# triq-org/spectroplot-js

Hardware: NVIDIA B200
Metric: Msamples/s rendered to RGBA spectrogram (N=4096) and % of B200 HBM roofline (higher is better)
Workload: dtype f32

## Files before the change

### spectroplot-js_b200/csrc/sp_kernel_r64.cuh

```cuda
#pragma once
#include "sp_prims.cuh"

#ifndef SP_XP
#define SP_XP 0
#endif
#ifndef SP_R64_TMA
#define SP_R64_TMA 1
#endif

namespace sp {

template <int FMT, bool SUB> struct R64Cfg {
    static constexpr int N = 4096, T = 64, STREAMS = 4, FFT_THREADS = T * STREAMS, STORE_THREADS = 128, THREADS = FFT_THREADS + STORE_THREADS;
    static constexpr int STEPS = 4, F = STREAMS * STEPS;
    static constexpr int FFT_REGS = 232, STORE_REGS = 40;
    static constexpr int SWB = SUB ? 8 : sample_width(FMT == FMT_RUNTIME ? CF64 : FMT);
    static constexpr bool OK = SUB || ((FMT != FMT_RUNTIME) && SWB <= 8);
    static constexpr int XP = 66;
    static constexpr int X_BYTES = 64 * XP * 8;
    static constexpr int WIN_PITCH = 64;
    static constexpr int TW_PITCH = 14;
    static constexpr int ST_PITCH = 1026;
    static constexpr int RING = 4;
    static constexpr bool TMA = SP_R64_TMA != 0;
    static constexpr int TILE_BYTES = TMA ? (STORE_THREADS / 32) * 4096 : 0;
    static constexpr size_t SMEM_BYTES = (size_t)STREAMS * X_BYTES + (size_t)F * ST_PITCH * 4 + (size_t)JH_SIZE * 4
                                       + ((SUB || TMA) ? 0 : (size_t)T * WIN_PITCH * 4) + TILE_BYTES + (size_t)T * TW_PITCH * 8 + 1024
                                       + (size_t)F * 2 * 8  + (size_t)2 * F * 8  + 192 + 1024 ;
    static_assert(SMEM_BYTES <= 232448, "render_r64_kernel: dynamic shared memory above the 227 KB an sm_100 CTA may have");
};

__device__ __forceinline__ unsigned lut_at(unsigned lut_base, unsigned word, int j)
{
    const unsigned a = ((j == 0 ? word << 2 : word >> (8 * j - 2)) & 0x3fcu) | lut_base;
    unsigned v;
    asm volatile("ld.shared.u32 %0, [%1];" : "=r"(v) : "r"(a));
    return v;
}

__device__ __forceinline__ void store_row8(uint32_t *rowp, uint4 a, uint4 b, bool aligned)
{
    if (aligned) st_global_256(rowp, a, b);
    else {
        rowp[0] = a.x; rowp[1] = a.y; rowp[2] = a.z; rowp[3] = a.w;
        rowp[4] = b.x; rowp[5] = b.y; rowp[6] = b.z; rowp[7] = b.w;
    }
}

__device__ __forceinline__ void stream_barrier(int stream)
{
    asm volatile("bar.sync %0, 64;" ::"r"(stream + 1) : "memory");
}

template <int FMT, bool SUB, bool OPT = false>
__global__ void __launch_bounds__(384, 1) render_r64_kernel(const Params p, const float2 *__restrict__ tw14, const __grid_constant__ CUtensorMap tmap)
{
    using B = R64Cfg<FMT, SUB>;
    constexpr int N = B::N, T = B::T, F = B::F;
    constexpr bool FLOAT_IN = SUB || FMT == CF32 || FMT == CF64 || FMT == FMT_RUNTIME;
    extern __shared__ __align__(128) unsigned char smem_r64[];
    const unsigned lut_base = (smem_u32(smem_r64) + 1023u) & ~1023u;
    unsigned char *s_x = smem_r64 + (lut_base - smem_u32(smem_r64)) + 1024;
    unsigned *s_lut = reinterpret_cast<unsigned *>(s_x - 1024);
    unsigned char *s_tiles = s_x + B::STREAMS * B::X_BYTES;
    unsigned *s_stage = reinterpret_cast<unsigned *>(s_tiles + B::TILE_BYTES);
    unsigned *s_jh = s_stage + F * B::ST_PITCH;
    float *s_win = reinterpret_cast<float *>(s_jh + JH_SIZE);
    float2 *s_tw = reinterpret_cast<float2 *>(s_win + ((SUB || B::TMA) ? 0 : T * B::WIN_PITCH));
    uint2 *s_mm = reinterpret_cast<uint2 *>(s_tw + T * B::TW_PITCH);
    float2 *s_fmid = reinterpret_cast<float2 *>(s_mm + F * 2);
    uint64_t *s_mbar = reinterpret_cast<uint64_t *>(s_fmid + 2 * F);
    int *s_off = reinterpret_cast<int *>(s_mbar + B::STREAMS);
    uint64_t *s_full = reinterpret_cast<uint64_t *>(s_off + B::STREAMS * 2);
    uint64_t *s_empty = s_full + 2;
    uint64_t *s_tready = s_empty + 2;
    long long *s_ring = reinterpret_cast<long long *>(s_tready + B::RING);
    long long *s_tile0 = s_ring + B::RING;

    const int tid = threadIdx.x;
    const int s = tid >> 6;
    const int t = tid & 63;
    float2 *X = reinterpret_cast<float2 *>(s_x + (size_t)s * B::X_BYTES);
    unsigned char *raw = reinterpret_cast<unsigned char *>(X);
    uint64_t *mbar = s_mbar + s;

    for (int i = tid; i < JH_SIZE; i += B::THREADS) s_jh[i] = 0;
    const int cmax = p.cmap_len - 1;
    const JhConst jc = jh_const(p);
    for (int i = tid; i < 256; i += B::THREADS) s_lut[i] = i <= cmax ? p.lut[jc.rev ? cmax - i : i] : 0u;
    for (int i = tid; i < T * B::TW_PITCH; i += B::THREADS) s_tw[i] = tw14[i];
    if constexpr (!SUB && !B::TMA)
        for (int i = tid; i < N; i += B::THREADS) s_win[(i & 63) * B::WIN_PITCH + (((i >> 6) + 4 * (i & 63)) & 63)] = p.window[i];
    const unsigned jh_base = smem_u32(s_jh) - (JH_MAGIC_BITS << 2);
    const int nfull = p.n_full, sub_r = p.sub_r;

    auto stage = [&](long long xr, int k0sub, unsigned par) {
        if (xr >= p.chunk_frames) xr = p.chunk_frames - 1;
        const void *src;
        unsigned bytes;
        if constexpr (SUB) {
            src = p.sub_in + ((size_t)xr * sub_r + (size_t)k0sub) * N;
            bytes = N * 8;
            s_off[s * 2 + par] = 0;
        } else {
            const long long xgl = p.frame_first + p.chunk_first + xr;
            const long long p0 = (long long)__dadd_rn(0.5, __dmul_rn(p.stride, (double)xgl)) - p.sample_base;
            const unsigned long long off = (unsigned long long)p0 * B::SWB, a0 = off & ~15ull;
            src = p.buf + a0;
            bytes = (unsigned)(((off - a0) + (unsigned long long)N * B::SWB + 15) & ~15ull);
            s_off[s * 2 + par] = (int)(off - a0);
        }
        tma_load_1d(raw, src, bytes, mbar);
    };
    auto tile_xr0 = [&](long long tile) -> long long { return (SUB ? tile / sub_r : tile) * F; };

    auto ticket = [&]() -> long long {
        const unsigned long long k = atomicAdd(p.tile_ctr, 1ull);
        if (k == (unsigned long long)p.ntiles + gridDim.x - 1) atomicExch(p.tile_ctr, 0ull);
        return (long long)k;
    };
    auto ring_put = [&](unsigned j, long long tl) {
        s_ring[(j - 1) % B::RING] = tl;
        mbar_arrive(s_tready + (j - 1) % B::RING);
    };
    auto ring_get = [&](unsigned j) -> long long {
        mbar_wait(s_tready + (j - 1) % B::RING, ((j - 1) / B::RING) & 1);
        return s_ring[(j - 1) % B::RING];
    };

    if (p.t_stamp && blockIdx.x == 0 && tid == 0) p.t_stamp[0] = globaltimer_ns();
    if (t == 0 && tid < B::FFT_THREADS) mbar_init(mbar, 1);
    if (tid == 0) {
        for (int h = 0; h < 2; h++) { mbar_init(s_full + h, B::FFT_THREADS / 32); mbar_init(s_empty + h, B::STORE_THREADS / 32); }
        for (int r = 0; r < B::RING; r++) mbar_init(s_tready + r, 1);
    }
    if (tid == B::FFT_THREADS) *s_tile0 = ticket();
    if (t == 0) asm volatile("fence.mbarrier_init.release.cluster;" ::: "memory");
    __syncthreads();
    long long tile = *s_tile0;
    unsigned kk = 0;

    if (tid >= B::FFT_THREADS) {
        asm volatile("setmaxnreg.dec.sync.aligned.u32 %0;" ::"n"(B::STORE_REGS));
        const int ht = tid - B::FFT_THREADS;
        const bool rows_aligned = (p.nframes % 8 == 0) && ((reinterpret_cast<uintptr_t>(p.image) & 31) == 0);
        if (ht == 0 && tile < p.ntiles) ring_put(1, ticket());
        griddep_wait();
        griddep_launch_dependents();
        while (tile < p.ntiles) {
            const int k0sub = SUB ? (int)(tile % sub_r) : 0;
            const long long xr0 = tile_xr0(tile);
#pragma unroll 1
            for (int h = 0; h < 2; h++) {
                mbar_wait(s_full + h, kk & 1);
                const size_t x0 = (size_t)(p.chunk_first + xr0) + 8 * h;
                const bool live = xr0 + 8 * h < p.chunk_frames;
                if constexpr (OPT && !SUB) {
                    if (p.waterfall && live) {
#pragma unroll 1
                        for (int f = 0; f < 8; f++) {
                            uint32_t *rowp = reinterpret_cast<uint32_t *>(p.image) + (size_t)N * (size_t)(p.nframes - 1 - (long long)(x0 + f));
                            const unsigned *src = s_stage + (8 * h + f) * B::ST_PITCH + ht;
#pragma unroll
                            for (int i = 0; i < 8; i++) {
                                const int id = ht + B::STORE_THREADS * i, k0 = id & 63, m = id >> 6;
                                const unsigned w = src[B::STORE_THREADS * i];
#pragma unroll
                                for (int j = 0; j < 4; j++)
                                    rowp[(k0 + 64 * (4 * m + j) + N / 2 - 1) & (N - 1)] = lut_at(lut_base, w, j);
                            }
                        }
                    }
                }
                if constexpr (B::TMA && !SUB) {
                    if (p.use_tma && live && (!OPT || !p.waterfall)) {
                        const int lane = ht & 31, wq = ht >> 5;
                        unsigned char *tile = s_tiles + wq * 4096;
                        const int r = 31 - lane;
                        const unsigned toff = (unsigned)(r * 32 + (((r >> 2) & 1) << 4));
#pragma unroll 1
                        for (int i = 0; i < 8; i++) {
                            const int id = ht + B::STORE_THREADS * i, k0 = id & 63, m = id >> 6;
                            const unsigned *src = s_stage + (8 * h) * B::ST_PITCH + m * 64 + k0;
                            unsigned w[8];
#pragma unroll
                            for (int f = 0; f < 8; f++) w[f] = src[f * B::ST_PITCH];
                            if (lane == 0) bulk_wait_read0();
                            __syncwarp();
#pragma unroll
                            for (int j = 0; j < 4; j++) {
                                uint4 a, b;
                                a.x = lut_at(lut_base, w[0], j); a.y = lut_at(lut_base, w[1], j); a.z = lut_at(lut_base, w[2], j); a.w = lut_at(lut_base, w[3], j);
                                b.x = lut_at(lut_base, w[4], j); b.y = lut_at(lut_base, w[5], j); b.z = lut_at(lut_base, w[6], j); b.w = lut_at(lut_base, w[7], j);
                                *reinterpret_cast<uint4 *>(tile + j * 1024 + toff) = a;
                                *reinterpret_cast<uint4 *>(tile + j * 1024 + (toff ^ 16u)) = b;
                                if (k0 + 64 * (4 * m + j) == N / 2)
                                    st_global_256(reinterpret_cast<uint32_t *>(p.image) + x0, a, b);
                            }
                            fence_async_smem();
                            __syncwarp();
                            if (lane == 0) {
                                const int kb0 = (k0 & 32) + 256 * m;
#pragma unroll
                                for (int j = 0; j < 4; j++)
                                    tma_store_2d(&tmap, smem_u32(tile + j * 1024), (int)x0, (N / 2 - (kb0 + 64 * j) - 31) & (N - 1));
                                bulk_commit();
                            }
                        }
                    }
                }
#pragma unroll 1
                for (int i = 0; i < ((live && (!OPT || SUB || !p.waterfall) && !(B::TMA && !SUB && p.use_tma)) ? 8 : 0); i++) {
                    const int id = ht + B::STORE_THREADS * i, k0 = id & 63, m = id >> 6;
                    const unsigned *src = s_stage + (8 * h) * B::ST_PITCH + m * 64 + k0;
                    unsigned w[8];
#pragma unroll
                    for (int f = 0; f < 8; f++) w[f] = src[f * B::ST_PITCH];
#pragma unroll
                    for (int j = 0; j < 4; j++) {
                        const int kb = k0 + 64 * (4 * m + j);
                        const int bin = SUB ? k0sub + sub_r * kb : kb;
                        const int y = (nfull / 2 - bin) & (nfull - 1);
                        uint32_t *rowp = reinterpret_cast<uint32_t *>(p.image) + (size_t)p.nframes * (size_t)y + x0;
                        uint4 a, b;
                        if (!(p.dbg & 4)) {
                            a.x = lut_at(lut_base, w[0], j); a.y = lut_at(lut_base, w[1], j); a.z = lut_at(lut_base, w[2], j); a.w = lut_at(lut_base, w[3], j);
                            b.x = lut_at(lut_base, w[4], j); b.y = lut_at(lut_base, w[5], j); b.z = lut_at(lut_base, w[6], j); b.w = lut_at(lut_base, w[7], j);
                        } else { a = make_uint4(w[0], w[1], w[2], w[3]); b = make_uint4(w[4], w[5], w[6], w[7]); }
                        if (!(p.dbg & 1)) store_row8(rowp, a, b, rows_aligned);
                    }
                }
                if (ht < 8 && live) {
                    const int fl = 8 * h + ht;
                    const long long xl = p.chunk_first + xr0 + fl;
                    const uint2 m0 = s_mm[fl * 2], m1 = s_mm[fl * 2 + 1];
                    const unsigned umn = min(m0.x, m1.x), umx = max(m0.y, m1.y);
                    const float mn = fminf(0.0f, fmaf(fast_log2(__uint_as_float(umn)), p.c1, p.c0));
                    const float mx = fmaxf(-200.0f, fmaf(fast_log2(__uint_as_float(umx)), p.c1, p.c0));
                    if constexpr (SUB) {
                        atomicMin(reinterpret_cast<unsigned *>(p.fmin) + xl, f2ord(mn));
                        atomicMax(reinterpret_cast<unsigned *>(p.fmax) + xl, f2ord(mx));
                    } else { p.fmin[xl] = mn; p.fmax[xl] = mx; p.fmid[xl] = s_fmid[(kk & 1) * F + fl]; }
                }
                __syncwarp();
                if ((ht & 31) == 0) mbar_arrive(s_empty + h);
            }
            tile = ring_get(++kk);
            if (ht == 0 && tile < p.ntiles) ring_put(kk + 1, ticket());
        }
        if constexpr (B::TMA && !SUB) bulk_wait_read0();
    } else {
    asm volatile("setmaxnreg.inc.sync.aligned.u32 %0;" ::"n"(B::FFT_REGS));
    unsigned fpar = 0;
    if (t == 0 && tile < p.ntiles) stage(tile_xr0(tile) + s, SUB ? (int)(tile % sub_r) : 0, 0);

    while (tile < p.ntiles) {
        const int k0sub = SUB ? (int)(tile % sub_r) : 0;
        const long long xr0 = tile_xr0(tile);
        long long next_tile = 0;

#pragma unroll 1
        for (int step = 0; step < B::STEPS; step++) {
            const int fl = step * B::STREAMS + s;
            const bool valid = xr0 + fl < p.chunk_frames;
            const unsigned jbase = valid ? jh_base : jh_base + (smem_u32(s_stage + 8 * B::ST_PITCH) - smem_u32(s_jh));
            int half = step >> 1;
            asm volatile("" : "+r"(half));
            if (step == B::STEPS - 1) next_tile = ring_get(kk + 1);
            cf v[64];
            const bool split = OPT && !SUB && p.channel_mode;
            auto prefetch = [&]() {
                if (step < B::STEPS - 1) stage(xr0 + fl + B::STREAMS, k0sub, fpar);
                else if (next_tile < p.ntiles) stage(tile_xr0(next_tile) + s, SUB ? (int)(next_tile % sub_r) : 0, fpar);
            };
            mbar_wait(mbar, fpar);
            if constexpr (SUB) {
#pragma unroll
                for (int n0 = 0; n0 < 8; n0++)
#pragma unroll
                    for (int n1 = 0; n1 < 8; n1++) v[8 * n1 + n0] = cld(reinterpret_cast<const float2 *>(raw) + T * (8 * n1 + n0) + t);
            } else {
                const unsigned char *rp = raw + s_off[s * 2 + fpar];
                const float4 *wrow = B::TMA ? p.window_t + t : reinterpret_cast<const float4 *>(s_win + t * B::WIN_PITCH);
#pragma unroll
                for (int qq = 0; qq < 16; qq++) {
                    const int q = 2 * (qq & 7) + (qq >> 3);
                    const float4 w = (SP_XP & 4) ? make_float4(1.f, 1.f, 1.f, 1.f) : B::TMA ? __ldg(wrow + 64 * q) : wrow[(q + t) & 15];
                    cf d[4];
#pragma unroll
                    for (int c = 0; c < 4; c++) d[c] = decode_raw_cf<FMT>(rp, T * (4 * q + c) + t, p.format);
                    if (q == 8 && t == 0 && valid) s_fmid[(kk & 1) * F + fl] = make_float2(cre(d[0]) * raw_scale<FMT>(), cim(d[0]) * raw_scale<FMT>());
                    v[4 * q] = cscale(d[0], w.x);     v[4 * q + 1] = cscale(d[1], w.y);
                    v[4 * q + 2] = cscale(d[2], w.z); v[4 * q + 3] = cscale(d[3], w.w);
                }
            }
            fpar ^= 1;
            dft64_between(v, [&] { stream_barrier(s); });
            {
                const float4 *twp = reinterpret_cast<const float4 *>(s_tw + t * B::TW_PITCH);
                float2 w[8];
                const float4 a = twp[0], b = twp[1], c = twp[2], d = twp[3];
                w[1] = make_float2(a.x, a.y); w[2] = make_float2(a.z, a.w); w[3] = make_float2(b.x, b.y); w[4] = make_float2(b.z, b.w);
                w[5] = make_float2(c.x, c.y); w[6] = make_float2(c.z, c.w); w[7] = make_float2(d.x, d.y);
#pragma unroll
                for (int j = 1; j < 8; j++) v[j] = cmul(v[j], w[j]);
#pragma unroll
                for (int j = 0; j < 8; j++) cst(X + j * B::XP + t, v[j]);
                float2 hi[8];
                hi[1] = make_float2(d.z, d.w);
                const float4 e = twp[4], f = twp[5], g = twp[6];
                hi[2] = make_float2(e.x, e.y); hi[3] = make_float2(e.z, e.w); hi[4] = make_float2(f.x, f.y);
                hi[5] = make_float2(f.z, f.w); hi[6] = make_float2(g.x, g.y); hi[7] = make_float2(g.z, g.w);
#pragma unroll
                for (int i = 1; i < 8; i++) {
                    v[8 * i] = cmul(v[8 * i], hi[i]);
#pragma unroll
                    for (int j = 1; j < 8; j++) v[8 * i + j] = cmul(v[8 * i + j], (SP_XP & 8) ? w[j] : cun(cmul(cpk(hi[i]), w[j])));
#pragma unroll
                    for (int j = 0; j < 8; j++) cst(X + (8 * i + j) * B::XP + t, v[8 * i + j]);
                }
            }
            stream_barrier(s);
            {
                const float4 *row = reinterpret_cast<const float4 *>(X + t * B::XP);
#pragma unroll
                for (int mm = 0; mm < 32; mm++) {
                    const int m = 4 * (mm & 7) + (mm >> 3);
                    const float4 q = row[m];
                    v[2 * m] = cpk(q.x, q.y); v[2 * m + 1] = cpk(q.z, q.w);
                }
            }
            dft64_between(v, [&] {
                stream_barrier(s);
                if (t == 0 && !split) prefetch();
            });
            if ((step & 1) == 0) mbar_wait(s_empty + half, (kk + 1) & 1);
            {
                {
                    if constexpr (OPT && !SUB) {
                        if (split) {
                            auto split_lo = [](cf a, cf b) {
                                const float2 fb = cun(b);
                                return cscale(cadd(a, cpk(fb.x, -fb.y)), 0.5f);
                            };
                            auto split_hi = [](cf a, cf b) {
                                const float2 fa = cun(a), fb = cun(b);
                                return cscale(cadd(cpk(fa.y, fa.x), cpk(fb.y, -fb.x)), 0.5f);
                            };
                            {
                                float4 *wrow = reinterpret_cast<float4 *>(X + t * B::XP);
#pragma unroll
                                for (int m = 0; m < 32; m++) {
                                    const float2 a = cun(v[2 * m]), b = cun(v[2 * m + 1]);
                                    wrow[m] = make_float4(a.x, a.y, b.x, b.y);
                                }
                            }
                            stream_barrier(s);
                            if (t == 0) {
#pragma unroll
                                for (int k1 = 1; k1 < 32; k1++) {
                                    const cf a = v[k1], b = v[64 - k1];
                                    v[k1] = split_lo(a, b);
                                    v[64 - k1] = split_hi(b, a);
                                }
                                v[0] = cpk(fmaf(0.0f, cim(v[0]), cre(v[0])), 0.0f);
                                v[32] = cpk(0.0f, 0.0f);
                            } else {
                                const float4 *prow = reinterpret_cast<const float4 *>(X + (64 - t) * B::XP);
#pragma unroll
                                for (int a = 0; a < 32; a++) {
                                    const float4 q = prow[31 - a];
                                    if (a < 16) {
                                        v[2 * a] = split_lo(v[2 * a], cpk(q.z, q.w));
                                        v[2 * a + 1] = split_lo(v[2 * a + 1], cpk(q.x, q.y));
                                    } else {
                                        v[2 * a] = split_hi(v[2 * a], cpk(q.z, q.w));
                                        v[2 * a + 1] = split_hi(v[2 * a + 1], cpk(q.x, q.y));
                                    }
                                }
                            }
                            stream_barrier(s);
                            if (t == 0) prefetch();
                        }
                    }

                    float amin = __int_as_float(0x7f800000), amax = 0.0f, prev = 0.0f;
                    unsigned umin_i = 0x7f800000u, umax_i = 0u;
                    unsigned *stg = s_stage + fl * B::ST_PITCH + t;
#pragma unroll
                    for (int m = 0; m < 16; m++) {
                        unsigned yb[4];
#pragma unroll
                        for (int j = 0; j < 4; j++) {
                            const float2 vi = cun(v[4 * m + j]);
                            const float abs2 = fmaf(vi.x, vi.x, vi.y * vi.y);
                            if constexpr (FLOAT_IN) {
                                umin_i = min(umin_i, __float_as_uint(abs2));
                                umax_i = max(umax_i, __float_as_uint(abs2));
                            } else if (j & 1) {
                                amin = fmin3(amin, prev, abs2);
                                amax = fmax3(amax, prev, abs2);
                            } else prev = abs2;
                            const float l2 = (SP_XP & 16) ? abs2 : fast_log2(abs2);
                            float Y;
                            const float S = (SP_XP & 16) ? (Y = l2, __uint_as_float((__float_as_uint(l2) >> 20) + JH_MAGIC_BITS)) : jh_eval(l2, jc, Y);
                            if constexpr ((SP_XP & 1) != 0) red_shared_inc_addr(smem_u32(s_jh) + ((tid & 31) << 2) + (__float_as_uint(S) & 0x380u));
                            else if constexpr (!(SP_XP & 2)) red_shared_inc_addr(jbase + (__float_as_uint(S) << 2));
                            yb[j] = __float_as_uint(Y);
                        }
                        stg[m * 64] = __byte_perm(__byte_perm(yb[0], yb[1], 0x0040), __byte_perm(yb[2], yb[3], 0x0040), 0x5410);
                    }
                    unsigned umn, umx;
                    if constexpr (FLOAT_IN) {
                        umn = __reduce_min_sync(0xffffffffu, umin_i);
                        umx = __reduce_max_sync(0xffffffffu, umax_i);
                    } else {
                        umn = __reduce_min_sync(0xffffffffu, __float_as_uint(amin));
                        umx = __reduce_max_sync(0xffffffffu, __float_as_uint(amax));
                    }
                    if (umn < 0x00800000u || umx >= 0x7f800000u) {
                        unsigned nzero = 0, nbad = 0, nnan = 0;
                        float mn = __int_as_float(0x7f800000), mx = 0.0f;
#pragma unroll
                        for (int i = 0; i < 64; i++) {
                            const float2 vi = cun(v[i]);
                            const float abs2 = fmaf(vi.x, vi.x, vi.y * vi.y);
                            nzero += abs2 < 1.17549435e-38f ? 1u : 0u;
                            nbad += !(abs2 <= 3.402823466e38f) ? 1u : 0u;
                            nnan += abs2 != abs2 ? 1u : 0u;
                            mn = fminf(mn, abs2 < 1.17549435e-38f ? 0.0f : abs2);
                            mx = fmaxf(mx, abs2);
                        }
                        nzero = __reduce_add_sync(0xffffffffu, nzero);
                        nbad = __reduce_add_sync(0xffffffffu, nbad);
                        nnan = __reduce_add_sync(0xffffffffu, nnan);
                        umn = __reduce_min_sync(0xffffffffu, __float_as_uint(mn));
                        umx = __reduce_max_sync(0xffffffffu, __float_as_uint(mx));
                        if ((t & 31) == 0 && valid) {
                            if (nzero) atomicAdd(&s_jh[JH_ZERO], nzero);
                            if (nbad) atomicAdd(&s_jh[JH_BAD], nbad);
                            if (nnan) {
                                float Yn;
                                const float Sn = jh_eval(__int_as_float(0x7fffffff), jc, Yn);
                                atomicSub(&s_jh[__float_as_uint(Sn) - JH_MAGIC_BITS], nnan);
                                atomicAdd(&s_jh[JH_NAN], nnan);
                            }
                        }
                    }
                    if ((t & 31) == 0) s_mm[fl * 2 + (t >> 5)] = make_uint2(umn, umx);
                    if (step & 1) {
                        __syncwarp();
                        if ((t & 31) == 0) mbar_arrive(s_full + half);
                    }
                }
            }
        }
        tile = next_tile;
        kk++;
    }
    }

    __syncthreads();
    griddep_wait();
    for (int i = tid; i < JH_SIZE; i += B::THREADS)
        if (s_jh[i]) atomicAdd(&p.j_hist[i], (unsigned long long)s_jh[i]);
}

}
```

Measured before the change: 422,900.

## Offload log/histogram epilogue to a dedicated epilogue warpgroup via smem hand-off

For non-subframe inputs with sample width up to 4 bytes, the FFT warps now write |X|^2 into a reserved tail of each stream's X buffer and signal an mbarrier. A new 128-thread epilogue warpgroup reads those values and does the log2, histogram increments, byte packing into the staging tile and min/max reduction. Per-chunk 'xfree' barriers let the FFT warps overwrite the hand-off area only once it has been consumed. The goal is to overlap the epilogue with the next frame's FFT and to lower FFT register pressure (192 instead of 232). The cost is more threads per CTA, extra mbarrier synchronisation and extra shared-memory traffic.

```diff
diff --git a/spectroplot-js_b200/csrc/sp_kernel_r64.cuh b/spectroplot-js_b200/csrc/sp_kernel_r64.cuh
--- a/spectroplot-js_b200/csrc/sp_kernel_r64.cuh
+++ b/spectroplot-js_b200/csrc/sp_kernel_r64.cuh
@@ -11,13 +11,17 @@
 namespace sp {
 
 template <int FMT, bool SUB> struct R64Cfg {
-    static constexpr int N = 4096, T = 64, STREAMS = 4, FFT_THREADS = T * STREAMS, STORE_THREADS = 128, THREADS = FFT_THREADS + STORE_THREADS;
+    static constexpr int N = 4096, T = 64, STREAMS = 4, FFT_THREADS = T * STREAMS, STORE_THREADS = 128;
     static constexpr int STEPS = 4, F = STREAMS * STEPS;
-    static constexpr int FFT_REGS = 232, STORE_REGS = 40;
     static constexpr int SWB = SUB ? 8 : sample_width(FMT == FMT_RUNTIME ? CF64 : FMT);
     static constexpr bool OK = SUB || ((FMT != FMT_RUNTIME) && SWB <= 8);
     static constexpr int XP = 66;
     static constexpr int X_BYTES = 64 * XP * 8;
+    static constexpr bool EPI_WG = !SUB && SWB <= 4;
+    static constexpr int XA_OFF = X_BYTES - 16 * 64 * 16;
+    static_assert(!EPI_WG || XA_OFF >= N * SWB + 32, "render_r64_kernel: the |X|^2 hand-off overlaps the raw frame");
+    static constexpr int EPI_THREADS = EPI_WG ? 32 * STREAMS : 0, THREADS = FFT_THREADS + STORE_THREADS + EPI_THREADS;
+    static constexpr int FFT_REGS = EPI_WG ? 192 : 232, STORE_REGS = 40, EPI_REGS = 88;
     static constexpr int WIN_PITCH = 64;
     static constexpr int TW_PITCH = 14;
     static constexpr int ST_PITCH = 1026;
@@ -26,7 +30,7 @@
     static constexpr int TILE_BYTES = TMA ? (STORE_THREADS / 32) * 4096 : 0;
     static constexpr size_t SMEM_BYTES = (size_t)STREAMS * X_BYTES + (size_t)F * ST_PITCH * 4 + (size_t)JH_SIZE * 4
                                        + ((SUB || TMA) ? 0 : (size_t)T * WIN_PITCH * 4) + TILE_BYTES + (size_t)T * TW_PITCH * 8 + 1024
-                                       + (size_t)F * 2 * 8  + (size_t)2 * F * 8  + 192 + 1024 ;
+                                       + (size_t)F * 2 * 8  + (size_t)2 * F * 8  + 384 + 1024 ;
     static_assert(SMEM_BYTES <= 232448, "render_r64_kernel: dynamic shared memory above the 227 KB an sm_100 CTA may have");
 };
 
@@ -52,8 +56,78 @@
     asm volatile("bar.sync %0, 64;" ::"r"(stream + 1) : "memory");
 }
 
+__device__ __forceinline__ float abs2_of(cf v)
+{
+    const float2 vi = cun(v);
+    return fmaf(vi.x, vi.x, vi.y * vi.y);
+}
+
+template <bool FLOAT_IN, int K, class Stg>
+__device__ __forceinline__ uint2 epi_bins(const float4 (&a)[K], Stg stg, const JhConst &jc, unsigned jbase, unsigned *s_jh, bool valid)
+{
+    float amin = __int_as_float(0x7f800000), amax = 0.0f, prev = 0.0f;
+    unsigned umin_i = 0x7f800000u, umax_i = 0u;
+#pragma unroll
+    for (int k = 0; k < K; k++) {
+        const float x[4] = {a[k].x, a[k].y, a[k].z, a[k].w};
+        unsigned yb[4];
+#pragma unroll
+        for (int j = 0; j < 4; j++) {
+            const float abs2 = x[j];
+            if constexpr (FLOAT_IN) {
+                umin_i = min(umin_i, __float_as_uint(abs2));
+                umax_i = max(umax_i, __float_as_uint(abs2));
+            } else if (j & 1) {
+                amin = fmin3(amin, prev, abs2);
+                amax = fmax3(amax, prev, abs2);
+            } else prev = abs2;
+            const float l2 = (SP_XP & 16) ? abs2 : fast_log2(abs2);
+            float Y;
+            const float S = (SP_XP & 16) ? (Y = l2, __uint_as_float((__float_as_uint(l2) >> 20) + JH_MAGIC_BITS)) : jh_eval(l2, jc, Y);
+            if constexpr ((SP_XP & 1) != 0) red_shared_inc_addr(smem_u32(s_jh) + ((threadIdx.x & 31) << 2) + (__float_as_uint(S) & 0x380u));
+            else if constexpr (!(SP_XP & 2)) red_shared_inc_addr(jbase + (__float_as_uint(S) << 2));
+            yb[j] = __float_as_uint(Y);
+        }
+        *stg(k) = __byte_perm(__byte_perm(yb[0], yb[1], 0x0040), __byte_perm(yb[2], yb[3], 0x0040), 0x5410);
+    }
+    unsigned umn = FLOAT_IN ? umin_i : __float_as_uint(amin), umx = FLOAT_IN ? umax_i : __float_as_uint(amax);
+    if (__any_sync(0xffffffffu, umn < 0x00800000u || umx >= 0x7f800000u)) {
+        unsigned nzero = 0, nbad = 0, nnan = 0;
+        float mn = __int_as_float(0x7f800000), mx = 0.0f;
+#pragma unroll
+        for (int k = 0; k < K; k++) {
+            const float x[4] = {a[k].x, a[k].y, a[k].z, a[k].w};
+#pragma unroll
+            for (int j = 0; j < 4; j++) {
+                const float abs2 = x[j];
+                nzero += abs2 < 1.17549435e-38f ? 1u : 0u;
+                nbad += !(abs2 <= 3.402823466e38f) ? 1u : 0u;
+                nnan += abs2 != abs2 ? 1u : 0u;
+                mn = fminf(mn, abs2 < 1.17549435e-38f ? 0.0f : abs2);
+                mx = fmaxf(mx, abs2);
+            }
+        }
+        nzero = __reduce_add_sync(0xffffffffu, nzero);
+        nbad = __reduce_add_sync(0xffffffffu, nbad);
+        nnan = __reduce_add_sync(0xffffffffu, nnan);
+        if ((threadIdx.x & 31) == 0 && valid) {
+            if (nzero) atomicAdd(&s_jh[JH_ZERO], nzero);
+            if (nbad) atomicAdd(&s_jh[JH_BAD], nbad);
+            if (nnan) {
+                float Yn;
+                const float Sn = jh_eval(__int_as_float(0x7fffffff), jc, Yn);
+                atomicSub(&s_jh[__float_as_uint(Sn) - JH_MAGIC_BITS], nnan);
+                atomicAdd(&s_jh[JH_NAN], nnan);
+            }
+        }
+        umn = __float_as_uint(mn);
+        umx = __float_as_uint(mx);
+    }
+    return make_uint2(umn, umx);
+}
+
 template <int FMT, bool SUB, bool OPT = false>
-__global__ void __launch_bounds__(384, 1) render_r64_kernel(const Params p, const float2 *__restrict__ tw14, const __grid_constant__ CUtensorMap tmap)
+__global__ void __launch_bounds__(R64Cfg<FMT, SUB>::THREADS, 1) render_r64_kernel(const Params p, const float2 *__restrict__ tw14, const __grid_constant__ CUtensorMap tmap)
 {
     using B = R64Cfg<FMT, SUB>;
     constexpr int N = B::N, T = B::T, F = B::F;
@@ -76,6 +150,8 @@
     uint64_t *s_tready = s_empty + 2;
     long long *s_ring = reinterpret_cast<long long *>(s_tready + B::RING);
     long long *s_tile0 = s_ring + B::RING;
+    uint64_t *s_xready = reinterpret_cast<uint64_t *>(s_tile0 + 1);
+    uint64_t *s_xfree = s_xready + B::STREAMS;
 
     const int tid = threadIdx.x;
     const int s = tid >> 6;
@@ -92,6 +168,7 @@
     if constexpr (!SUB && !B::TMA)
         for (int i = tid; i < N; i += B::THREADS) s_win[(i & 63) * B::WIN_PITCH + (((i >> 6) + 4 * (i & 63)) & 63)] = p.window[i];
     const unsigned jh_base = smem_u32(s_jh) - (JH_MAGIC_BITS << 2);
+    auto jbase_of = [&](bool valid) { return valid ? jh_base : jh_base + (smem_u32(s_stage + 8 * B::ST_PITCH) - smem_u32(s_jh)); };
     const int nfull = p.n_full, sub_r = p.sub_r;
 
     auto stage = [&](long long xr, int k0sub, unsigned par) {
@@ -129,9 +206,15 @@
     };
 
     if (p.t_stamp && blockIdx.x == 0 && tid == 0) p.t_stamp[0] = globaltimer_ns();
-    if (t == 0 && tid < B::FFT_THREADS) mbar_init(mbar, 1);
+    if (t == 0 && tid < B::FFT_THREADS) {
+        mbar_init(mbar, 1);
+        if constexpr (B::EPI_WG) {
+            mbar_init(s_xready + s, 2);
+            for (int c = 0; c < 4; c++) mbar_init(s_xfree + 4 * s + c, 1);
+        }
+    }
     if (tid == 0) {
-        for (int h = 0; h < 2; h++) { mbar_init(s_full + h, B::FFT_THREADS / 32); mbar_init(s_empty + h, B::STORE_THREADS / 32); }
+        for (int h = 0; h < 2; h++) { mbar_init(s_full + h, B::EPI_WG ? B::STREAMS : B::FFT_THREADS / 32); mbar_init(s_empty + h, B::STORE_THREADS / 32); }
         for (int r = 0; r < B::RING; r++) mbar_init(s_tready + r, 1);
     }
     if (tid == B::FFT_THREADS) *s_tile0 = ticket();
@@ -140,7 +223,7 @@
     long long tile = *s_tile0;
     unsigned kk = 0;
 
-    if (tid >= B::FFT_THREADS) {
+    if (tid >= B::FFT_THREADS && tid < B::FFT_THREADS + B::STORE_THREADS) {
         asm volatile("setmaxnreg.dec.sync.aligned.u32 %0;" ::"n"(B::STORE_REGS));
         const int ht = tid - B::FFT_THREADS;
         const bool rows_aligned = (p.nframes % 8 == 0) && ((reinterpret_cast<uintptr_t>(p.image) & 31) == 0);
@@ -233,7 +316,7 @@
                 if (ht < 8 && live) {
                     const int fl = 8 * h + ht;
                     const long long xl = p.chunk_first + xr0 + fl;
-                    const uint2 m0 = s_mm[fl * 2], m1 = s_mm[fl * 2 + 1];
+                    const uint2 m0 = s_mm[fl * 2], m1 = B::EPI_WG ? m0 : s_mm[fl * 2 + 1];
                     const unsigned umn = min(m0.x, m1.x), umx = max(m0.y, m1.y);
                     const float mn = fminf(0.0f, fmaf(fast_log2(__uint_as_float(umn)), p.c1, p.c0));
                     const float mx = fmaxf(-200.0f, fmaf(fast_log2(__uint_as_float(umx)), p.c1, p.c0));
@@ -249,9 +332,55 @@
             if (ht == 0 && tile < p.ntiles) ring_put(kk + 1, ticket());
         }
         if constexpr (B::TMA && !SUB) bulk_wait_read0();
+    } else if (tid >= B::FFT_THREADS + B::STORE_THREADS) {
+        if constexpr (B::EPI_WG) {
+        asm volatile("setmaxnreg.dec.sync.aligned.u32 %0;" ::"n"(B::EPI_REGS));
+        const int lane = tid & 31, es = (tid - B::FFT_THREADS - B::STORE_THREADS) >> 5;
+        const float4 *xa = reinterpret_cast<const float4 *>(s_x + (size_t)es * B::X_BYTES + B::XA_OFF) + lane;
+        unsigned xpar = 0;
+        while (tile < p.ntiles) {
+            const long long xr0 = tile_xr0(tile);
+            long long next_tile = 0;
+#pragma unroll 1
+            for (int step = 0; step < B::STEPS; step++) {
+                const int fl = step * B::STREAMS + es;
+                const bool valid = xr0 + fl < p.chunk_frames;
+                const unsigned jbase = jbase_of(valid);
+                int half = step >> 1;
+                asm volatile("" : "+r"(half));
+                if (step == B::STEPS - 1) next_tile = ring_get(kk + 1);
+                if ((step & 1) == 0) mbar_wait(s_empty + half, (kk + 1) & 1);
+                mbar_wait(s_xready + es, xpar);
+                xpar ^= 1;
+                unsigned umn = 0xffffffffu, umx = 0u;
+#pragma unroll 1
+                for (int c = 0; c < 4; c++) {
+                    float4 a[8];
+#pragma unroll
+                    for (int k = 0; k < 8; k++) a[k] = xa[(4 * c + (k >> 1)) * 64 + 32 * (k & 1)];
+                    __syncwarp();
+                    if (lane == 0) mbar_arrive(s_xfree + 4 * es + c);
+                    const uint2 mm = epi_bins<FLOAT_IN>(a, [&](int k) { return s_stage + fl * B::ST_PITCH + (4 * c + (k >> 1)) * 64 + 32 * (k & 1) + lane; },
+                                                        jc, jbase, s_jh, valid);
+                    umn = min(umn, mm.x);
+                    umx = max(umx, mm.y);
+                }
+                umn = __reduce_min_sync(0xffffffffu, umn);
+                umx = __reduce_max_sync(0xffffffffu, umx);
+                if (lane == 0) s_mm[fl * 2] = make_uint2(umn, umx);
+                if (step & 1) {
+                    __syncwarp();
+                    if (lane == 0) mbar_arrive(s_full + half);
+                }
+            }
+            tile = next_tile;
+            kk++;
+        }
+        }
     } else {
     asm volatile("setmaxnreg.inc.sync.aligned.u32 %0;" ::"n"(B::FFT_REGS));
     unsigned fpar = 0;
+    bool handed = false;
     if (t == 0 && tile < p.ntiles) stage(tile_xr0(tile) + s, SUB ? (int)(tile % sub_r) : 0, 0);
 
     while (tile < p.ntiles) {
@@ -263,7 +392,6 @@
         for (int step = 0; step < B::STEPS; step++) {
             const int fl = step * B::STREAMS + s;
             const bool valid = xr0 + fl < p.chunk_frames;
-            const unsigned jbase = valid ? jh_base : jh_base + (smem_u32(s_stage + 8 * B::ST_PITCH) - smem_u32(s_jh));
             int half = step >> 1;
             asm volatile("" : "+r"(half));
             if (step == B::STEPS - 1) next_tile = ring_get(kk + 1);
@@ -313,6 +441,7 @@
                 hi[5] = make_float2(f.z, f.w); hi[6] = make_float2(g.x, g.y); hi[7] = make_float2(g.z, g.w);
 #pragma unroll
                 for (int i = 1; i < 8; i++) {
+                    if (B::EPI_WG && i >= 4 && handed) mbar_wait(s_xfree + 4 * s + (i - 4), fpar);
                     v[8 * i] = cmul(v[8 * i], hi[i]);
 #pragma unroll
                     for (int j = 1; j < 8; j++) v[8 * i + j] = cmul(v[8 * i + j], (SP_XP & 8) ? w[j] : cun(cmul(cpk(hi[i]), w[j])));
@@ -334,7 +463,7 @@
                 stream_barrier(s);
                 if (t == 0 && !split) prefetch();
             });
-            if ((step & 1) == 0) mbar_wait(s_empty + half, (kk + 1) & 1);
+            if (!B::EPI_WG && (step & 1) == 0) mbar_wait(s_empty + half, (kk + 1) & 1);
             {
                 {
                     if constexpr (OPT && !SUB) {
@@ -384,73 +513,27 @@
                         }
                     }
 
-                    float amin = __int_as_float(0x7f800000), amax = 0.0f, prev = 0.0f;
-                    unsigned umin_i = 0x7f800000u, umax_i = 0u;
-                    unsigned *stg = s_stage + fl * B::ST_PITCH + t;
-#pragma unroll
-                    for (int m = 0; m < 16; m++) {
-                        unsigned yb[4];
-#pragma unroll
-                        for (int j = 0; j < 4; j++) {
-                            const float2 vi = cun(v[4 * m + j]);
-                            const float abs2 = fmaf(vi.x, vi.x, vi.y * vi.y);
-                            if constexpr (FLOAT_IN) {
-                                umin_i = min(umin_i, __float_as_uint(abs2));
-                                umax_i = max(umax_i, __float_as_uint(abs2));
-                            } else if (j & 1) {
-                                amin = fmin3(amin, prev, abs2);
-                                amax = fmax3(amax, prev, abs2);
-                            } else prev = abs2;
-                            const float l2 = (SP_XP & 16) ? abs2 : fast_log2(abs2);
-                            float Y;
-                            const float S = (SP_XP & 16) ? (Y = l2, __uint_as_float((__float_as_uint(l2) >> 20) + JH_MAGIC_BITS)) : jh_eval(l2, jc, Y);
-                            if constexpr ((SP_XP & 1) != 0) red_shared_inc_addr(smem_u32(s_jh) + ((tid & 31) << 2) + (__float_as_uint(S) & 0x380u));
-                            else if constexpr (!(SP_XP & 2)) red_shared_inc_addr(jbase + (__float_as_uint(S) << 2));
-                            yb[j] = __float_as_uint(Y);
+                    if constexpr (B::EPI_WG) {
+                        float4 *xa = reinterpret_cast<float4 *>(raw + B::XA_OFF) + t;
+#pragma unroll
+                        for (int m = 0; m < 16; m++)
+                            xa[m * 64] = make_float4(abs2_of(v[4 * m]), abs2_of(v[4 * m + 1]), abs2_of(v[4 * m + 2]), abs2_of(v[4 * m + 3]));
+                        handed = true;
+                        __syncwarp();
+                        if ((t & 31) == 0) mbar_arrive(s_xready + s);
+                    } else {
+                        float4 a2[16];
+#pragma unroll
+                        for (int m = 0; m < 16; m++)
+                            a2[m] = make_float4(abs2_of(v[4 * m]), abs2_of(v[4 * m + 1]), abs2_of(v[4 * m + 2]), abs2_of(v[4 * m + 3]));
+                        const uint2 mm = epi_bins<FLOAT_IN>(a2, [&](int m) { return s_stage + fl * B::ST_PITCH + t + 64 * m; }, jc,
+                                                            jbase_of(valid), s_jh, valid);
+                        const unsigned umn = __reduce_min_sync(0xffffffffu, mm.x), umx = __reduce_max_sync(0xffffffffu, mm.y);
+                        if ((t & 31) == 0) s_mm[fl * 2 + (t >> 5)] = make_uint2(umn, umx);
+                        if (step & 1) {
+                            __syncwarp();
+                            if ((t & 31) == 0) mbar_arrive(s_full + half);
                         }
-                        stg[m * 64] = __byte_perm(__byte_perm(yb[0], yb[1], 0x0040), __byte_perm(yb[2], yb[3], 0x0040), 0x5410);
-                    }
-                    unsigned umn, umx;
-                    if constexpr (FLOAT_IN) {
-                        umn = __reduce_min_sync(0xffffffffu, umin_i);
-                        umx = __reduce_max_sync(0xffffffffu, umax_i);
-                    } else {
-                        umn = __reduce_min_sync(0xffffffffu, __float_as_uint(amin));
-                        umx = __reduce_max_sync(0xffffffffu, __float_as_uint(amax));
-                    }
-                    if (umn < 0x00800000u || umx >= 0x7f800000u) {
-                        unsigned nzero = 0, nbad = 0, nnan = 0;
-                        float mn = __int_as_float(0x7f800000), mx = 0.0f;
-#pragma unroll
-                        for (int i = 0; i < 64; i++) {
-                            const float2 vi = cun(v[i]);
-                            const float abs2 = fmaf(vi.x, vi.x, vi.y * vi.y);
-                            nzero += abs2 < 1.17549435e-38f ? 1u : 0u;
-                            nbad += !(abs2 <= 3.402823466e38f) ? 1u : 0u;
-                            nnan += abs2 != abs2 ? 1u : 0u;
-                            mn = fminf(mn, abs2 < 1.17549435e-38f ? 0.0f : abs2);
-                            mx = fmaxf(mx, abs2);
-                        }
-                        nzero = __reduce_add_sync(0xffffffffu, nzero);
-                        nbad = __reduce_add_sync(0xffffffffu, nbad);
-                        nnan = __reduce_add_sync(0xffffffffu, nnan);
-                        umn = __reduce_min_sync(0xffffffffu, __float_as_uint(mn));
-                        umx = __reduce_max_sync(0xffffffffu, __float_as_uint(mx));
-                        if ((t & 31) == 0 && valid) {
-                            if (nzero) atomicAdd(&s_jh[JH_ZERO], nzero);
-                            if (nbad) atomicAdd(&s_jh[JH_BAD], nbad);
-                            if (nnan) {
-                                float Yn;
-                                const float Sn = jh_eval(__int_as_float(0x7fffffff), jc, Yn);
-                                atomicSub(&s_jh[__float_as_uint(Sn) - JH_MAGIC_BITS], nnan);
-                                atomicAdd(&s_jh[JH_NAN], nnan);
-                            }
-                        }
-                    }
-                    if ((t & 31) == 0) s_mm[fl * 2 + (t >> 5)] = make_uint2(umn, umx);
-                    if (step & 1) {
-                        __syncwarp();
-                        if ((t & 31) == 0) mbar_arrive(s_full + half);
                     }
                 }
             }
```

After: 406,300 (median of 6 runs). 0.961x the previous value.
